# nianticlabs/implicit-depth

Measured on AMD Instinct MI355X. Metric: frames/sec (BDModel.forward hot path, 512x384, 64 planes, 8-frame tuple = 1 current + 7 source views; third-party backbones excluded), higher is better.
Workload: dtype f32

## Files before the change

implicit-depth_amd/csrc/model.hip:

```cpp
#include <cstring>
#include <vector>

#include "idh_common.h"
#include "net_plan.h"
#include "../../include/idh_model.h"

namespace {

using idh_internal::ConvStage;

constexpr int kAbi = 106;
constexpr int kHidden = 128;
constexpr int kMaxCols = 256;

inline size_t align64(size_t v) { return (v + 63) & ~(size_t)63; }

struct ColMap {
    int n;
    int col[kMaxCols];
};

__global__ __launch_bounds__(256) void pack_cols_k(const float *__restrict__ w, int ld, ColMap cols, float *__restrict__ dst, int cblocks) {
    const int total = cblocks * (kHidden / 16) * 64 * 4;
    for (int t = blockIdx.x * 256 + threadIdx.x; t < total; t += gridDim.x * 256) {
// ... 106 lines not shown
    }
    return IDH_OK;
}

uint64_t fnv(uint64_t h, const void *p, size_t n) {
    const unsigned char *c = static_cast<const unsigned char *>(p);
    for (size_t i = 0; i < n; ++i) { h ^= c[i]; h *= 1099511628211ull; }
    return h;
}

void stage_of(const idh_model_desc *d, int B, const idh_model_inputs *in, float *const *log_depth, float *const *depth, ConvStage &cs) {
    const idh_model_params *n = d->net;
    cs = ConvStage{};
    cs.enc = n->cv_blocks; cs.n_enc = 4; cs.dec = n->dec_blocks;
    cs.heads = d->kind == IDH_MODEL_DEPTH ? n->depth_heads : nullptr;
    cs.N = B; cs.H = d->H; cs.W = d->W; cs.D = d->D;
    int h = d->H, w = d->W;
    for (int i = 0; i < 4; ++i) {
        const int st = n->cv_blocks[3 * i].conv1.stride;
        if (st == 1 || st == 2) { h = (h + 2 - 3) / st + 1; w = (w + 2 - 3) / st + 1; }
        const int cimg = n->cv_blocks[3 * i + 1].conv1.cin - n->cv_blocks[3 * i].conv1.cout;
        cs.img[i + 1] = idh_tensor{in ? const_cast<float *>(in->pyramid[i + 1]) : nullptr, IDH_LAYOUT_NCHW, cimg, h, w, 0};
    }
    cs.img[0] = idh_tensor{in ? const_cast<float *>(in->pyramid[0]) : nullptr, IDH_LAYOUT_NCHW, n->dec_blocks[14].conv1.cin, 2 * cs.img[1].H, 2 * cs.img[1].W, 0};
    cs.log_depth = log_depth; cs.depth = depth;
    cs.head_mode = d->matching_input == IDH_MATCH_LAYER1_NCHW ? 1 : d->matching_input == IDH_MATCH_LAYER1_NHWC ? 2 : 0;
    cs.K = d->K;
    cs.head = n->match_head;
    cs.layer1 = in ? in->matching_layer1 : nullptr;
}
// ... 328 lines not shown
```

implicit-depth_amd/csrc/net_plan.h:

```cpp
#pragma once
#include <stddef.h>
#include <stdint.h>

#include "idh_common.h"
#include "../../include/idh_net.h"

namespace idh_internal {

enum { STAGE_SIZES = 0, STAGE_PACK = 1, STAGE_RUN = 2 };

struct ConvStage {
    const idh_block_params *enc;
    int n_enc;
    const idh_block_params *dec;
    const idh_conv_params *heads;
    int N, H, W, D;
    idh_tensor img[5];
    float *const *log_depth;
    float *const *depth;
    int head_mode;
    int K;
    const idh_conv_params *head;
    const float *layer1;
    float *cv_in;
    int cv_cs;
    const float *feat0;
    int feat0_cs, feat0_C, feat0_H, feat0_W;
    const float *match;
    int n_head_ops;
    int level_H[5], level_W[5];
// ... 12 lines not shown
```

implicit-depth_amd/csrc/networks.hip:

```cpp
#include <algorithm>
#include <array>
#include <cstring>
#include <map>
#include <tuple>
#include <vector>

#include "idh_common.h"
#include "net_plan.h"
#include "../../include/idh_net.h"
#include "../../include/idh_ops.h"

namespace {

constexpr int kWinoMinTiles = 128;
constexpr double kWinoMinFill = 0.74;
constexpr int kWino4MinTiles = 768;
constexpr double kWino4MinFill = 0.85;
constexpr long long kReuseMinBytes = 64ll << 20;
constexpr int kNarrowTileBelow = 400;
constexpr int kSplitMinChunks = 6, kSplitMax = 16;
constexpr double kProjChunkWeight = 0.5;
constexpr int kS2FirstMinBlocks = 512;
constexpr int kTargetWaves = 2048, kMinWaves = 1024;
constexpr int kTileWino = IDH_TILE_WINO, kTileWino4 = IDH_TILE_WINO4;
// ... 66 lines not shown

    float *ws_alloc(size_t floats) {
        float *p = ws_ + ws_off;
        ws_off = align64(ws_off + floats);
        if (mode_ == MODE_RUN && ws_off > ws_cap_) err = IDH_EWORKSPACE;
        return p;
    }
    float *blob_alloc(size_t floats) {
        float *p = blob_ + blob_off;
        blob_off = align64(blob_off + floats);
        return p;
    }

    View buffer(int n, int h, int w, int c) {
        const int cs_ = ceil16(c);
        if (cs_ == c) {
            auto it = free_.find(std::make_tuple(n, h, w, cs_));
            if (it != free_.end() && !it->second.empty()) {
                const int b = it->second.back();
                it->second.pop_back();
                ++recycled;
                return View{b, 0, c};
            }
        }
        Buf b{};
        b.N = n; b.H = h; b.W = w; b.cs = cs_; b.internal = true; b.zero_fill = cs_ != c;
        b.floats = (size_t)n * h * w * cs_;
        b.base = ws_alloc(b.floats);
        bufs.push_back(b);
        return View{(int)bufs.size() - 1, 0, c};
    }
    View external(const idh_tensor &t, int n) {
        Buf b{};
        b.N = n; b.H = t.H; b.W = t.W; b.cs = t.cs; b.internal = false; b.zero_fill = false;
        b.base = mode_ == MODE_RUN ? t.ptr : reinterpret_cast<float *>((uintptr_t(2) << 32) + ((uintptr_t)bufs.size() << 24));
        bufs.push_back(b);
        return View{(int)bufs.size() - 1, 0, t.C};
    }
    void release(const View &v) {
        const Buf &b = bufs[v.buf];
        if (!b.internal || v.c0 != 0 || v.C != b.cs || (long long)b.floats * 4 < kReuseMinBytes) return;
        auto &pool = free_[std::make_tuple(b.N, b.H, b.W, b.cs)];
        if (std::find(pool.begin(), pool.end(), v.buf) != pool.end()) { err = IDH_EINVAL; return; }
// ... 125 lines not shown
            if (v.C != c.cin || (c.ks != 1 && c.ks != 3) || c.cout != cout) { err = IDH_EINVAL; return out; }
            if (v.C % 16 && (v.c0 != 0 || cs(v) != ceil16(v.C))) { err = IDH_EINVAL; return out; }
            const WLayout lay = (use_wino4 && i == 0) ? W_WINO4 : (use_wino && i == 0) ? W_WINO : W_DIRECT;
            idh_conv_src &s = op.src[i];
            s.in = ptr(v); s.w = packed(c, lay); s.cs = cs(v); s.H = H(v); s.W = W(v); s.Cin = v.C;
            s.ks = c.ks; s.stride = c.stride; s.pad_mode = pad_mode;
            steps += c.ks * c.ks * (ceil16(v.C) / 16);
        }
        op.bias = bias_of(cv, cv2);
        if (res) { op.res = ptr(*res); op.res_cs = cs(*res); }
        op.out = ptr(out); op.out_cs = cs(out);
        op.Ho = Ho; op.Wo = Wo; op.Cout = cout;
        op.act = act; op.slope = slope;
        const long long M = (long long)n * Ho * Wo;
        int tm, tn, split;
        if (use_wino4) { tm = kTileWino4; tn = 0; split = 1; ++n_wino4; }
        else if (use_wino) { tm = kTileWino; tn = 0; split = 1; ++n_wino2; }
        else if (lds_eligible(srcs, cout, Wo, pad_mode)) {
            double ch = 0;
            for (const Src &s : srcs) ch += (ceil16(s.v.C) / 16) * (s.cv->ks == 3 ? 1.0 : kProjChunkWeight);
            choose_lds_tile(n, Ho, Wo, cout, (int)ch, tm, split);
            tn = lds_subtiles(cout);
            if (tn == 4 && tm == 9 && kNarrowTileBelow) {
                const long long blocks64 = (long long)n * cdiv(Ho, 4) * cdiv(Wo, 16) * (cout / 64) * split;
                if (blocks64 < kNarrowTileBelow) tn = 2;
            }
            tn = tn == 4 ? 0 : tn;
        } else if (!norm && s2_first_eligible(srcs, cout, n, Ho, Wo, pad_mode)) {
            choose_lds_tile(n, Ho, Wo, cout, ceil16(x.C) / 16, tm, split);
            tn = lds_subtiles(cout);
            tn = tn == 4 ? 0 : tn;
        } else {
            choose_tiles(M, cout, steps, tm, tn, split);
        }
        op.tile_m = tm; op.tile_n = tn; op.split_k = split;
        if (norm) {
            if ((tm != 8 && tm != 9) || tn != 1 || x2) { err = IDH_EINVAL; return out; }
            op.src[0].norm = norm->stats; op.src[0].norm_act = norm->act; op.src[0].norm_slope = norm->slope;
        }
        if (split > 1) op.ws = ws_alloc((size_t)split * M * ceil16(cout));
        ops.push_back(op);
        Meta m;
        if (res) m.reads.push_back(region(*res));
        if (norm) m.reads.push_back(Region{norm->buf, 0, 1});
        for (const Src &s : srcs) m.reads.push_back(region(s.v, true));
        m.writes.push_back(region(out));
        meta.push_back(m);
        return out;
    }
    void upsample2(const View &x, const View &out) {
        if (err) return;
        idh_op op;
        std::memset(&op, 0, sizeof op);
        op.kind = IDH_OP_UPSAMPLE2; op.N = N(x);
// ... 112 lines not shown
        const int planes = blk.conv1.cout;
        const View h = buffer(N(x), Ho, Wo, planes);
        conv(x, blk.conv1, h, IDH_ACT_LRELU, 0.2f, nullptr, nullptr, nullptr);
        const View out = out_opt ? *out_opt : buffer(N(x), Ho, Wo, planes);
        if (H(out) != Ho || W(out) != Wo) { err = IDH_EINVAL; return out; }
        if (blk.downsample.ks == 0) {
            if (x.C != planes || st != 1) { err = IDH_EINVAL; return out; }
            conv(h, blk.conv2, out, IDH_ACT_LRELU, 0.2f, &x, nullptr, nullptr);
        } else {
            conv(h, blk.conv2, out, IDH_ACT_LRELU, 0.2f, nullptr, &x, &blk.downsample);
        }
        release(h);
        return out;
    }

    static bool overlap(const std::vector<Region> &a, const std::vector<Region> &b) {
        for (const Region &x : a)
            for (const Region &y : b)
                if (x.buf == y.buf && x.c0 < y.c1 && y.c0 < x.c1) return true;
        return false;
    }
    static void launch_rank(const idh_op &op, long long r[3]) {
        r[0] = 3; r[1] = 0; r[2] = 0;
        if (op.kind == IDH_OP_CONV && op.tile_m == kTileWino) { r[0] = -1; r[1] = op.src[1].in ? 1 : 0; r[2] = -(long long)op.N * op.Ho * op.Wo * op.Cout; }
        else if (op.kind == IDH_OP_CONV && op.tile_m == 9) { r[0] = 0; r[1] = op.tile_n; }
        else if (op.kind == IDH_OP_CONV && op.tile_m == 1 && op.tile_n == 4) { r[0] = 1; }
        else if (op.kind == IDH_OP_UPSAMPLE2) { r[0] = 2; }
        else if (op.kind == IDH_OP_NCHW_TO_NHWC) { r[0] = 2; r[1] = 1; }
    }
    void schedule(int n_first = 0) {
// ... 38 lines not shown
        }
        return IDH_OK;
    }

    Mode mode() const { return mode_; }
    hipStream_t stream() const { return st_; }
    int (*before_run)(void *) = nullptr;
    void *before_ctx = nullptr;

  private:
    Mode mode_;
    float *ws_;
    size_t ws_cap_;
    float *blob_;
    hipStream_t st_;
    std::map<std::tuple<int, int, int, int>, std::vector<int>> free_;
};

bool tensor_ok(const idh_tensor *t, bool need_ptr, bool read = true) {
    if (!t || t->C <= 0 || t->H <= 0 || t->W <= 0) return false;
    if (t->layout != IDH_LAYOUT_NHWC && t->layout != IDH_LAYOUT_NCHW) return false;
    if (t->layout == IDH_LAYOUT_NHWC && (t->cs < t->C || (t->cs & 3) || (read && (t->C & 15) && t->cs != ceil16(t->C)))) return false;
    if (need_ptr && (!t->ptr || ((uintptr_t)t->ptr & 15))) return false;
    return true;
}

View input_view(Plan &p, const idh_tensor &t, int N) {
    if (t.layout == IDH_LAYOUT_NHWC) return p.external(t, N);
    const View v = p.buffer(N, t.H, t.W, t.C);
    p.import_nchw(t.ptr, N, t.C, t.H, t.W, v);
// ... 86 lines not shown
        }
        if (levels) levels->push_back(y);
        x = y;
        if (p.err) return p.err;
    }
    return p.err;
}

int build_cvencoder(Plan &p, const idh_block_params *blocks, int num_blocks, int N, const idh_tensor *cost, const idh_tensor *img, const idh_tensor *outs) {
    const bool run = p.mode() == MODE_RUN;
    if (!blocks || num_blocks <= 0 || num_blocks > 8 || N <= 0 || !tensor_ok(cost, run) || !img || !outs) return IDH_EINVAL;
    return cvencoder_body(p, blocks, num_blocks, N, input_view(p, *cost, N), img, outs, nullptr);
}

int unetpp_body(Plan &p, const idh_block_params *blocks, const idh_conv_params *heads, int N, std::vector<View> prev, const idh_tensor *fouts,
                float *const *log_depth, float *const *depth, View *feat0) {
    const bool run = p.mode() == MODE_RUN;
    const idh_block_params *out_blk[4] = {nullptr, &blocks[46], &blocks[47], &blocks[48]};
    auto want = [&](int i) { return fouts && fouts[i].C > 0; };
    std::vector<View> outputs;
    View final_v[4];
    int bi = 0;
    for (int j = 1; j <= 4; ++j) {
        for (int i = 4 - j; i >= 0; --i) {
            const idh_block_params &right = blocks[bi++], &diag = blocks[bi++];
            const bool has_up = (i + j) != 4;
            const idh_block_params *up = has_up ? &blocks[bi++] : nullptr;
            const idh_block_params &in0 = blocks[bi++], &in1 = blocks[bi++];
            const int cout = right.conv1.cout;
            const View xi = prev[i];
            const View cat = p.buffer(N, p.H(xi), p.W(xi), cout * (has_up ? 3 : 2));
            const View s0 = Plan::slice(cat, 0, cout);
            p.basic_block(xi, right, &s0);
            const View lo = p.basic_block(prev[i + 1], diag);
            if (p.H(lo) * 2 != p.H(xi) || p.W(lo) * 2 != p.W(xi)) return IDH_EINVAL;
            p.upsample2(lo, Plan::slice(cat, cout, cout));
            p.release(lo);
            if (has_up) {
                const View lo2 = p.basic_block(outputs.back(), *up);
                p.upsample2(lo2, Plan::slice(cat, 2 * cout, cout));
                p.release(lo2);
            }
            const View y0 = p.basic_block(cat, in0);
            p.release(cat);
            const bool last = j == 4 - i;
            View y;
            if (last && i == 0 && want(0) && fouts[0].layout == IDH_LAYOUT_NHWC) {
                if (!tensor_ok(&fouts[0], run) || fouts[0].C != in1.conv1.cout) return IDH_EINVAL;
                const View o = p.external(fouts[0], N);
                y = p.basic_block(y0, in1, &o);
            } else {
                y = p.basic_block(y0, in1);
                if (last && i == 0 && want(0)) {
                    if (!tensor_ok(&fouts[0], run) || fouts[0].C != in1.conv1.cout) return IDH_EINVAL;
                    p.export_nchw(y, fouts[0].ptr);
                }
            }
            p.release(y0);
            outputs.push_back(y);
            if (last) {
                if (i == 0) final_v[0] = y;
                else if (want(i)) {
                    if (!tensor_ok(&fouts[i], run) || fouts[i].C != out_blk[i]->conv1.cout) return IDH_EINVAL;
                    const View o = output_view(p, fouts[i], N);
                    final_v[i] = p.basic_block(y, *out_blk[i], &o);
                    output_done(p, fouts[i], final_v[i]);
                } else if (heads) {
                    final_v[i] = p.basic_block(y, *out_blk[i]);
                }
            }
            if (p.err) return p.err;
        }
        prev.assign(outputs.rbegin(), outputs.rend());
    }
    if (heads) {
        for (int i = 0; i < 4; ++i) {
            if (run && (!log_depth || !log_depth[i])) return IDH_EINVAL;
            p.head(final_v[i], heads[i], run ? log_depth[i] : nullptr, (run && depth) ? depth[i] : nullptr);
        }
    }
    if (feat0) *feat0 = final_v[0];
    return p.err;
}

int build_unetpp(Plan &p, const idh_block_params *blocks, int n_blocks, const idh_conv_params *heads, int N, const idh_tensor *feats,
                 const idh_tensor *fouts, float *const *log_depth, float *const *depth) {
    const bool run = p.mode() == MODE_RUN;
    if (!blocks || n_blocks != IDH_UNETPP_BLOCKS || N <= 0 || !feats) return IDH_EINVAL;
    std::vector<View> prev;
    for (int i = 0; i < 5; ++i) {
        if (!tensor_ok(&feats[i], run)) return IDH_EINVAL;
        if (i && (feats[i].H * 2 != feats[i - 1].H || feats[i].W * 2 != feats[i - 1].W)) return IDH_EINVAL;
        prev.push_back(input_view(p, feats[i], N));
    }
    return unetpp_body(p, blocks, heads, N, prev, fouts, log_depth, depth, nullptr);
}

uint64_t layout_hash(const std::vector<idh_op> &ops) {
    uint64_t h = 1469598103934665603ull;
    auto mix = [&](long long v) {
        for (int i = 0; i < 8; ++i) { h ^= (uint64_t)((v >> (8 * i)) & 0xff); h *= 1099511628211ull; }
    };
    for (const idh_op &op : ops) {
        mix(op.kind); mix(op.N); mix(op.Ho); mix(op.Wo); mix(op.Cout); mix(op.tile_m); mix(op.tile_n); mix(op.split_k); mix(op.act); mix(op.group);
        for (const idh_conv_src &s : op.src) { mix(s.Cin); mix(s.H); mix(s.W); mix(s.cs); mix(s.ks); mix(s.stride); mix(s.pad_mode); mix(s.norm != nullptr); }
    }
    return h;
}

}
// ... 42 lines not shown
        if (p.err) return p.err;
        if (p.cs(mo) != mo.C) return IDH_EUNSUPPORTED;
        s->match = p.ptr(mo);
        s->n_head_ops = (int)p.ops.size();
    }
    const View cv_in = p.buffer(s->N, s->H, s->W, s->D);
    for (int i = 0; i < 5; ++i)
        if (s->img[i].layout != IDH_LAYOUT_NCHW || !tensor_ok(&s->img[i], m == MODE_RUN)) return IDH_EINVAL;
    const View v0 = input_view(p, s->img[0], s->N);
    std::vector<View> levels{v0};
    int rc = cvencoder_body(p, s->enc, s->n_enc, s->N, cv_in, &s->img[1], nullptr, &levels);
    if (rc != IDH_OK) return rc;
    for (int i = 1; i < 5; ++i)
        if (p.H(levels[i]) * 2 != p.H(levels[i - 1]) || p.W(levels[i]) * 2 != p.W(levels[i - 1])) return IDH_EINVAL;
    View f0;
    rc = unetpp_body(p, s->dec, s->heads, s->N, levels, nullptr, s->log_depth, s->depth, &f0);
    if (rc != IDH_OK) return rc;
    s->cv_in = p.ptr(cv_in);
    s->cv_cs = p.cs(cv_in);
    s->feat0 = p.ptr(f0);
    s->feat0_cs = p.cs(f0); s->feat0_C = f0.C; s->feat0_H = p.H(f0); s->feat0_W = p.W(f0);
    for (int i = 0; i < 5; ++i) { s->level_H[i] = p.H(levels[i]); s->level_W[i] = p.W(levels[i]); }
    p.before_run = before_ops;
    p.before_ctx = ctx;
    idh_net_sizes sz{};
    if (m == MODE_PACK) return p.err;
    rc = p.finish(m == MODE_SIZES ? &sz : nullptr, s->n_head_ops);
    if (rc != IDH_OK) return rc;
    if (m == MODE_SIZES) {
        s->ws_floats = sz.workspace_floats; s->weight_floats = sz.weight_floats; s->ops = sz.ops; s->launches = sz.launches;
        s->layout_hash = layout_hash(p.ops);
// ... 54 lines not shown
                               const idh_tensor *feature_outs, float *blob, void *stream) {
    if (!blob || ((uintptr_t)blob & 255)) return IDH_EINVAL;
    Plan p(MODE_PACK, nullptr, 0, blob, idh_stream(stream));
    const int rc = build_unetpp(p, blocks, n_blocks, heads, N, feats, feature_outs, nullptr, nullptr);
    return rc != IDH_OK ? rc : p.err;
}
extern "C" int idh_unetpp_fwd(const idh_block_params *blocks, int n_blocks, const idh_conv_params *heads, const float *blob, int N,
                              const idh_tensor *feats, const idh_tensor *feature_outs, float *const *log_depth_outs, float *const *depth_outs,
                              float *ws, size_t ws_floats, void *stream) {
    if (!blob || ((uintptr_t)blob & 255) || !ws || ((uintptr_t)ws & 255)) return IDH_EINVAL;
    Plan p(MODE_RUN, ws, ws_floats, const_cast<float *>(blob), idh_stream(stream));
    const int rc = build_unetpp(p, blocks, n_blocks, heads, N, feats, feature_outs, log_depth_outs, depth_outs);
    return rc != IDH_OK ? rc : p.finish(nullptr);
}

extern "C" int idh_matching_stem_sizes(const idh_stem_params *params, int N, const idh_tensor *images, const idh_tensor *out, idh_net_sizes *sizes) {
    if (!sizes) return IDH_EINVAL;
    Plan p(MODE_SIZES, nullptr, 0, nullptr, nullptr);
    const int rc = build_matching_stem(p, params, N, images, out);
    return rc != IDH_OK ? rc : p.finish(sizes);
}
extern "C" int idh_matching_stem_pack(const idh_stem_params *params, int N, const idh_tensor *images, const idh_tensor *out, float *blob, void *stream) {
    if (!blob || ((uintptr_t)blob & 255)) return IDH_EINVAL;
    Plan p(MODE_PACK, nullptr, 0, blob, idh_stream(stream));
    const int rc = build_matching_stem(p, params, N, images, out);
    return rc != IDH_OK ? rc : p.err;
}
extern "C" int idh_matching_stem_fwd(const idh_stem_params *params, const float *blob, int N, const idh_tensor *images, const idh_tensor *out, float *ws,
                                     size_t ws_floats, void *stream) {
    if (!blob || ((uintptr_t)blob & 255) || !ws || ((uintptr_t)ws & 255)) return IDH_EINVAL;
// ... 5 lines not shown
```

implicit-depth_amd/net_abi.py:

```python
from __future__ import annotations

import ctypes as C
from typing import List, Optional, Sequence

import torch
from torch import nn

from . import _lib

LAYOUT_NHWC, LAYOUT_NCHW = 0, 1
UNETPP_BLOCKS = 49


class Tensor(C.Structure):
    _fields_ = [("ptr", C.c_void_p), ("layout", C.c_int32), ("C", C.c_int32), ("H", C.c_int32), ("W", C.c_int32), ("cs", C.c_int32)]


class ConvParams(C.Structure):
    _fields_ = [("weight", C.c_void_p), ("bias", C.c_void_p), ("cout", C.c_int32), ("cin", C.c_int32), ("ks", C.c_int32), ("stride", C.c_int32)]


class BlockParams(C.Structure):
    _fields_ = [("conv1", ConvParams), ("conv2", ConvParams), ("downsample", ConvParams)]


class NetSizes(C.Structure):
# ... 87 lines not shown


def _sigs():
    P = C.POINTER
    vp, i32, sz = C.c_void_p, C.c_int, C.c_size_t
    return {
        "idh_basic_block_sizes": (i32, [P(BlockParams), i32, P(Tensor), P(Tensor), P(NetSizes)]),
        "idh_basic_block_pack": (i32, [P(BlockParams), i32, P(Tensor), P(Tensor), vp, vp]),
        "idh_basic_block_fwd": (i32, [P(BlockParams), vp, i32, P(Tensor), P(Tensor), vp, sz, vp]),
        "idh_cvencoder_sizes": (i32, [P(BlockParams), i32, i32, P(Tensor), P(Tensor), P(Tensor), P(NetSizes)]),
        "idh_cvencoder_pack": (i32, [P(BlockParams), i32, i32, P(Tensor), P(Tensor), P(Tensor), vp, vp]),
        "idh_cvencoder_fwd": (i32, [P(BlockParams), i32, vp, i32, P(Tensor), P(Tensor), P(Tensor), vp, sz, vp]),
        "idh_unetpp_sizes": (i32, [P(BlockParams), i32, P(ConvParams), i32, P(Tensor), P(Tensor), P(NetSizes)]),
        "idh_unetpp_pack": (i32, [P(BlockParams), i32, P(ConvParams), i32, P(Tensor), P(Tensor), vp, vp]),
        "idh_unetpp_fwd": (i32, [P(BlockParams), i32, P(ConvParams), vp, i32, P(Tensor), P(Tensor), P(vp), P(vp), vp, sz, vp]),
        "idh_matching_stem_sizes": (i32, [P(StemParams), i32, P(Tensor), P(Tensor), P(NetSizes)]),
        "idh_matching_stem_pack": (i32, [P(StemParams), i32, P(Tensor), P(Tensor), vp, vp]),
        "idh_matching_stem_fwd": (i32, [P(StemParams), vp, i32, P(Tensor), P(Tensor), vp, sz, vp]),
    }


SIGS = _sigs()


def tensors(ts: Sequence[Tensor]):
    return (Tensor * len(ts))(*ts)


def ptr_array(ts: Optional[List[torch.Tensor]]):
    if ts is None:
# ... 3 lines not shown
```

implicit-depth_amd/nhwc.py:

```python
from __future__ import annotations

import ctypes as C
from dataclasses import dataclass
from typing import Dict, List, Optional, Sequence

import torch
from torch import nn

from . import _lib

OP_CONV, OP_UPSAMPLE2, OP_IMPORT, OP_EXPORT, OP_SPLITK, OP_HEAD, OP_INSTNORM, OP_UPSAMPLE2_NEAREST, OP_COPY, OP_POINTWISE_NCHW, OP_POINTWISE_UP = 1, 2, 3, 4, 5, 6, 7, 8, 9, 10, 11
OP_STEM = 12
ACT_NONE, ACT_LRELU, ACT_ELU = 0, 1, 2
PAD_ZEROS, PAD_REPLICATE = 0, 1


class ConvSrc(C.Structure):
    _fields_ = [("in_", C.c_void_p), ("w", C.c_void_p), ("cs", C.c_int32), ("H", C.c_int32), ("W", C.c_int32),
                ("Cin", C.c_int32), ("ks", C.c_int32), ("stride", C.c_int32), ("pad_mode", C.c_int32), ("_r", C.c_int32),
                ("up_in", C.c_void_p * 2), ("up_cs", C.c_int32 * 2), ("up_c0", C.c_int32), ("up_C", C.c_int32),
                ("norm", C.c_void_p), ("norm_slope", C.c_float), ("norm_act", C.c_int32)]


class Op(C.Structure):
# ... 904 lines not shown
        i_out = [p.export_nchw(o) for o in outs]
        p.schedule()
        ent = (p, i_x, i_img, i_out, outs)
        cache.put(key, ent)
    p, i_x, i_img, i_out, outs = ent
    res = [torch.empty(o.N, o.C, o.H, o.W, device=x.device, dtype=torch.float32) for o in outs]
    p.set_in(i_x, x)
    for i, f in zip(i_img, img_feats):
        p.set_in(i, f)
    for i, r in zip(i_out, res):
        p.set_out(i, r)
    p.run()
    return res


def build_decoder(p: Plan, dec, feats: List[View]):
    prev = list(feats)
    outputs: List[View] = []
    final: Dict[int, View] = {}
    for j in range(1, 5):
        for i in range(4 - j, -1, -1):
            right = dec.convs[f"right_conv_{i}{j - 1}"]
            diag = dec.convs[f"diag_conv_{i + 1}{j - 1}"]
            cout = right.conv1.out_channels
            has_up = (i + j) != 4
            xi = prev[i]
            seq = dec.convs[f"in_conv_{i}{j}"]
            fuse = (FUSE_UPSAMPLE and p.math == "fp32" and cout % 16 == 0 and xi.W >= 16 and
                    lds_eligible([(xi, seq[0].conv1)], seq[0].conv1.out_channels, xi.W, PAD_ZEROS) and seq[0].downsample is not None and
                    seq[0].downsample[0].kernel_size[0] == 1)
            if fuse:
                r = p.basic_block(xi, right)
                lo = p.basic_block(prev[i + 1], diag)
                if (lo.H * 2, lo.W * 2) != (xi.H, xi.W):
                    raise _lib.IdhError("decoder pyramid levels must differ by exactly x2")
                ups = [lo] + ([p.basic_block(outputs[-1], dec.convs[f"up_conv_{i + 1}{j}"])] if has_up else [])
                cat = CatView(r, ups)
            else:
                cat = p.buffer(xi.N, xi.H, xi.W, cout * (3 if has_up else 2))
                p.basic_block(xi, right, out=cat.slice(0, cout))
                lo = p.basic_block(prev[i + 1], diag)
                if (lo.H * 2, lo.W * 2) != (xi.H, xi.W):
                    raise _lib.IdhError("decoder pyramid levels must differ by exactly x2")
                p.upsample2(lo, cat.slice(cout, cout))
                lows = [lo]
                hold_lows = PROJ_LOWRES
                if not hold_lows:
                    p.release(lo)
                if has_up:
                    lo2 = p.basic_block(outputs[-1], dec.convs[f"up_conv_{i + 1}{j}"])
                    p.upsample2(lo2, cat.slice(2 * cout, cout))
                    lows.append(lo2)
                    if not hold_lows:
                        p.release(lo2)
            y0 = p.basic_block_upcat(cat, lows, seq[0]) if isinstance(cat, View) else None
            if y0 is None:
                y0 = p.basic_block(cat, seq[0])
            if isinstance(cat, View):
                if hold_lows:
                    for l in lows:
                        p.release(l)
                p.release(cat)
            y = p.basic_block(y0, seq.conv_0)
            p.release(y0)
            outputs.append(y)
            if j == 4 - i:
                head = dec.convs[f"output_{i}"]
                final[i] = p.basic_block(y, head[0]) if not isinstance(head[0], nn.Identity) else y
        prev = outputs[::-1]
    return final


def decoder_forward_nchw(dec, input_features: List[torch.Tensor]) -> Dict[str, torch.Tensor]:
    _check_in(*input_features)
    feats = [f.contiguous() for f in input_features]
    key = ("dec", tuple(tuple(f.shape) for f in feats), str(feats[0].device), _param_key(dec))
    cache = _plan_cache(dec)
    ent = cache.get(key)
    if ent is None:
        p = Plan(feats[0].device, math=math_of(dec))
        views, i_in = [], []
        for f in feats:
            v = p.buffer(f.shape[0], f.shape[2], f.shape[3], f.shape[1])
# ... 226 lines not shown
    final: Dict[int, View] = {}
    for bi, blk in enumerate((dec.block1, dec.block2, dec.block3, dec.block4)):
        skip = feats[-2 - bi]
        cout = blk.pre_concat_conv.conv2.out_channels
        y = _conv_block(p, x, blk.pre_concat_conv)
        if (y.H * 2, y.W * 2) != (skip.H, skip.W):
            raise _lib.IdhError("decoder pyramid levels must differ by exactly x2")
        cat = p.buffer(skip.N, skip.H, skip.W, cout + skip.C)
        p.upsample2(y, cat.slice(0, cout), nearest=True)
        p.copy(skip, cat.slice(cout, skip.C))
        x = _conv_block(p, cat, blk.post_concat_conv)
        final[3 - bi] = x
    return final


def build_any_decoder(p: Plan, dec, feats: List[View]) -> Dict[int, View]:
    if hasattr(dec, "block1"):
        return build_skip_decoder(p, dec, feats)
    return build_decoder(p, dec, feats)


def build_regression_heads(p: Plan, dec, final: Dict[int, View]) -> Dict[int, "tuple"]:
    heads = {}
    for i, seq in ((3, dec.out1), (2, dec.out2), (1, dec.out3), (0, dec.out4)):
        v = final[i]
        h1 = p.buffer(v.N, v.H, v.W, seq[0].out_channels)
        p.conv(v, seq[0], h1, act=ACT_ELU)
        h2 = p.buffer(v.N, v.H, v.W, seq[2].out_channels)
        p.conv(h1, seq[2], h2, act=ACT_ELU)
        heads[i] = (h2, seq[4])
    return heads


def skip_regression_forward_nchw(dec, input_features: List[torch.Tensor]) -> Dict[str, torch.Tensor]:
# ... 34 lines not shown
```

implicit-depth_amd/pipeline.py:

```python
from __future__ import annotations

from typing import Dict, List, Optional, Sequence

import torch
from torch import nn

from . import _lib, nhwc
from .cost_volume import CostVolumeManager, ZeroCostVolumeManager, volume_opts
from .mlp import occlusion_logits


class HotPath(nn.Module):

    def __init__(self, cost_volume: nn.Module, cost_volume_net: nn.Module, depth_decoder: nn.Module,
                 binary_mlp: Optional[nn.Module] = None, min_depth: float = 0.25, max_depth: float = 5.0,
                 conv_math: Optional[str] = None, matching_model: Optional[nn.Module] = None):
        super().__init__()
        self.conv_math = conv_math
        self.cost_volume = cost_volume
        self.cost_volume_net = cost_volume_net
        self.depth_decoder = depth_decoder
        self.binary_mlp = binary_mlp
        self.matching_model = matching_model
        self.min_depth, self.max_depth = float(min_depth), float(max_depth)
        self.thresholder = None
        self._plans = nhwc.PlanCache()
        _lib.watch_state_dict_loads(self)

    def _plan(self, B, K, C, H, W, enc_shapes: Sequence[Sequence[int]], device, head: Optional[str] = None, head_ch: int = 0,
              images: Optional[torch.Tensor] = None):
        geom = None
        if head == "images":
            _, shape, strides = nhwc.image_strides(images)
            geom = (tuple(shape), strides)
        key = (B, K, C, H, W, tuple(tuple(s) for s in enc_shapes), str(device), self.conv_math, head, head_ch, geom,
               nhwc._param_key(self.cost_volume_net), nhwc._param_key(self.depth_decoder),
               nhwc.ParamKey(nhwc._param_key(self.matching_model.net[5]) + nhwc._param_key(self.matching_model.net[8])) if head else None,
               nhwc.stem_param_key(self.matching_model.net[:5]) if head == "images" else None)
        ent = self._plans.get(key)
        if ent is not None:
            return ent
        D = self.cost_volume.num_depth_bins
        p = nhwc.Plan(device, math=self.conv_math)
        st = {"lowest": None, "planes": torch.empty(D, device=device)}
        ent = {"plan": p, "state": st, "heads": {}, "i_l1": None}
        if head is None:
            st["cur_n"] = torch.empty(B, H, W, C, device=device)
            st["src_n"] = torch.empty(B, K, H, W, C, device=device)
            ent["feats"] = (st["cur_n"].data_ptr(), st["src_n"].data_ptr(), (B, K, C, H, W), 0, 0)
        else:
# ... 11 lines not shown
            else:
                x = nhwc.View(torch.empty(1, device=device).expand(M, H, W, head_ch), 0, head_ch)
                y = nhwc.build_matching_head(p, self.matching_model, x)
                ent["i_l1"] = n0
            if y.C != C:
                raise _lib.IdhError(f"matching head produces {y.C} channels, cost volume expects {C}")
            hw = H * W * C
            ent["feats"] = (y.ptr, y.ptr + 4 * hw, (B, K, C, H, W), (K + 1) * hw, (K + 1) * hw)
            ent["match_view"] = y
        n_pre = len(p.ops)
        cv_in = p.buffer(B, H, W, D)
        v0 = p.buffer(B, enc_shapes[0][2], enc_shapes[0][3], enc_shapes[0][1])
        i_enc = [p.import_nchw(enc_shapes[0], v0)]
        outs, i_img = nhwc.build_cv_encoder(p, self.cost_volume_net, cv_in, enc_shapes[1:])
        i_enc += i_img
        final = nhwc.build_any_decoder(p, self.depth_decoder, [v0] + outs)
        ent.update(cv_in=cv_in, i_enc=i_enc, final=final)
        if getattr(self.depth_decoder, "depth_head", False):
            for i, v in final.items():
                ent["heads"][i] = p.head(v, self.depth_decoder.convs[f"output_{i}"][1], torch.empty(1, device=device))
        elif hasattr(self.depth_decoder, "out1"):
            for i, (hv, last) in nhwc.build_regression_heads(p, self.depth_decoder, final).items():
                ent["heads"][i] = p.head(hv, last, torch.empty(1, device=device))
        ent["n_head_ops"] = p.schedule_segments(n_pre)
        return self._plans.put(key, ent)

    def forward(self, matching_cur_feats: Optional[torch.Tensor], matching_src_feats: Optional[torch.Tensor], cur_feats: List[torch.Tensor],
                src_cam_T_cur_cam: torch.Tensor, cur_cam_T_src_cam: torch.Tensor, src_K: torch.Tensor, cur_invK: torch.Tensor,
                rendered_depth: Optional[torch.Tensor] = None, prior: Optional[torch.Tensor] = None,
                return_mask: bool = False, return_features: bool = False,
                prior_inputs: Optional[Dict[str, torch.Tensor]] = None, infer_depth: bool = False,
# ... 24 lines not shown
            if matching_layer1.dim() != 5:
                raise _lib.IdhError(f"matching_layer1 must be (B, K+1, C, H, W), got {tuple(matching_layer1.shape)}")
            B, K1, head_ch, H, W = matching_layer1.shape
            K, C = K1 - 1, self.matching_model.net[8].out_channels
            l1 = matching_layer1.reshape(B * K1, head_ch, H, W)
            if l1.is_contiguous():
                head = "nchw"
            elif l1.is_contiguous(memory_format=torch.channels_last):
                head = "nhwc"
            else:
                l1, head = l1.contiguous(), "nchw"
        else:
            B, K, C, H, W = matching_src_feats.shape
        dev = src_K.device
        cur_feats = [f if f.is_contiguous() else f.contiguous() for f in cur_feats]
        ent = self._plan(B, K, C, H, W, [f.shape for f in cur_feats], dev, head, head_ch, images)
        p, st = ent["plan"], ent["state"]
        L = _lib.lib()
        sp = _lib.stream_ptr()
        D = self.cost_volume.num_depth_bins
        out: Dict[str, torch.Tensor] = {}

        zero_volume = isinstance(self.cost_volume, ZeroCostVolumeManager)
        if head is not None:
            p.set_in(ent["i_l1"], l1)
            p.run(0, ent["n_head_ops"])
        elif not zero_volume:
            mc = matching_cur_feats if matching_cur_feats.is_contiguous() else matching_cur_feats.contiguous()
            ms = matching_src_feats if matching_src_feats.is_contiguous() else matching_src_feats.contiguous()
            _lib.check(L.idh_nchw_to_nhwc_f32(mc.data_ptr(), st["cur_n"].data_ptr(), B, C, H * W, sp), "idh_nchw_to_nhwc_f32")
            _lib.check(L.idh_nchw_to_nhwc_f32(ms.data_ptr(), st["src_n"].data_ptr(), B * K, C, H * W, sp), "idh_nchw_to_nhwc_f32")
# ... 94 lines not shown
```

include/idh_net.h:

```cpp
#ifndef IDH_NET_H_
#define IDH_NET_H_

#include <stddef.h>
#include <stdint.h>

#ifdef __cplusplus
extern "C" {
#endif
#if defined(__GNUC__) || defined(__clang__)
#pragma GCC visibility push(default)
#endif

#define IDH_LAYOUT_NHWC 0
#define IDH_LAYOUT_NCHW 1

typedef struct idh_tensor {
    float *ptr;
    int32_t layout;
    int32_t C, H, W;
    int32_t cs;
} idh_tensor;

typedef struct idh_conv_params {
    const float *weight;
// ... 23 lines not shown
                        const idh_tensor *outs, idh_net_sizes *sizes);
int idh_cvencoder_pack(const idh_block_params *blocks, int num_blocks, int N, const idh_tensor *cost, const idh_tensor *img_feats,
                       const idh_tensor *outs, float *weight_blob, void *stream);
int idh_cvencoder_fwd(const idh_block_params *blocks, int num_blocks, const float *weight_blob, int N, const idh_tensor *cost,
                      const idh_tensor *img_feats, const idh_tensor *outs, float *workspace, size_t workspace_floats, void *stream);

#define IDH_UNETPP_BLOCKS 49
int idh_unetpp_sizes(const idh_block_params *blocks, int n_blocks, const idh_conv_params *heads, int N, const idh_tensor *feats,
                     const idh_tensor *feature_outs, idh_net_sizes *sizes);
int idh_unetpp_pack(const idh_block_params *blocks, int n_blocks, const idh_conv_params *heads, int N, const idh_tensor *feats,
                    const idh_tensor *feature_outs, float *weight_blob, void *stream);
int idh_unetpp_fwd(const idh_block_params *blocks, int n_blocks, const idh_conv_params *heads, const float *weight_blob, int N,
                   const idh_tensor *feats, const idh_tensor *feature_outs, float *const *log_depth_outs, float *const *depth_outs,
                   float *workspace, size_t workspace_floats, void *stream);

typedef struct idh_bn_params {
    const float *weight, *bias, *running_mean, *running_var;
    float eps;
    int32_t _r;
} idh_bn_params;

typedef struct idh_stem_params {
    const float *conv1_weight;
    idh_bn_params bn1;
    const float *layer1_conv[4];
    idh_bn_params layer1_bn[4];
} idh_stem_params;

int idh_matching_stem_sizes(const idh_stem_params *params, int N, const idh_tensor *images, const idh_tensor *out, idh_net_sizes *sizes);
int idh_matching_stem_pack(const idh_stem_params *params, int N, const idh_tensor *images, const idh_tensor *out, float *weight_blob, void *stream);
// ... 11 lines not shown
```

Before: 680.9.

## Skip unused coarse-scale decoder output blocks and release low-res inputs early

Adds a scale mask to the UNet++ decoder so the output_i blocks for coarse scales are skipped when only the finest scale is consumed (non-depth model, or Python pipeline when no features are returned). A dry-run reservation path keeps weight-blob packing offsets stable while no kernels are emitted. It also releases intermediate pyramid inputs earlier, so workspace buffers can be recycled. The risk is that it drops outputs some callers may need when the mask is misapplied.

```diff
diff --git a/implicit-depth_amd/csrc/model.hip b/implicit-depth_amd/csrc/model.hip
--- a/implicit-depth_amd/csrc/model.hip
+++ b/implicit-depth_amd/csrc/model.hip
@@ -144,6 +144,7 @@
     cs = ConvStage{};
     cs.enc = n->cv_blocks; cs.n_enc = 4; cs.dec = n->dec_blocks;
     cs.heads = d->kind == IDH_MODEL_DEPTH ? n->depth_heads : nullptr;
+    cs.scales = d->kind == IDH_MODEL_DEPTH ? IDH_SCALES_ALL : 0x1;
     cs.N = B; cs.H = d->H; cs.W = d->W; cs.D = d->D;
     int h = d->H, w = d->W;
     for (int i = 0; i < 4; ++i) {
diff --git a/implicit-depth_amd/csrc/net_plan.h b/implicit-depth_amd/csrc/net_plan.h
--- a/implicit-depth_amd/csrc/net_plan.h
+++ b/implicit-depth_amd/csrc/net_plan.h
@@ -14,6 +14,7 @@
     int n_enc;
     const idh_block_params *dec;
     const idh_conv_params *heads;
+    unsigned scales;
     int N, H, W, D;
     idh_tensor img[5];
     float *const *log_depth;
diff --git a/implicit-depth_amd/csrc/networks.hip b/implicit-depth_amd/csrc/networks.hip
--- a/implicit-depth_amd/csrc/networks.hip
+++ b/implicit-depth_amd/csrc/networks.hip
@@ -104,6 +104,7 @@
 
     View buffer(int n, int h, int w, int c) {
         const int cs_ = ceil16(c);
+        if (dry_) return phantom(n, h, w, c, cs_);
         if (cs_ == c) {
             auto it = free_.find(std::make_tuple(n, h, w, cs_));
             if (it != free_.end() && !it->second.empty()) {
@@ -117,6 +118,13 @@
         b.N = n; b.H = h; b.W = w; b.cs = cs_; b.internal = true; b.zero_fill = cs_ != c;
         b.floats = (size_t)n * h * w * cs_;
         b.base = ws_alloc(b.floats);
+        bufs.push_back(b);
+        return View{(int)bufs.size() - 1, 0, c};
+    }
+    View phantom(int n, int h, int w, int c, int cs_) {
+        Buf b{};
+        b.N = n; b.H = h; b.W = w; b.cs = cs_; b.internal = false; b.zero_fill = false;
+        b.base = reinterpret_cast<float *>((uintptr_t(7) << 32) + ((uintptr_t)bufs.size() << 24));
         bufs.push_back(b);
         return View{(int)bufs.size() - 1, 0, c};
     }
@@ -272,8 +280,8 @@
         op.act = act; op.slope = slope;
         const long long M = (long long)n * Ho * Wo;
         int tm, tn, split;
-        if (use_wino4) { tm = kTileWino4; tn = 0; split = 1; ++n_wino4; }
-        else if (use_wino) { tm = kTileWino; tn = 0; split = 1; ++n_wino2; }
+        if (use_wino4) { tm = kTileWino4; tn = 0; split = 1; n_wino4 += !dry_; }
+        else if (use_wino) { tm = kTileWino; tn = 0; split = 1; n_wino2 += !dry_; }
         else if (lds_eligible(srcs, cout, Wo, pad_mode)) {
             double ch = 0;
             for (const Src &s : srcs) ch += (ceil16(s.v.C) / 16) * (s.cv->ks == 3 ? 1.0 : kProjChunkWeight);
@@ -296,6 +304,7 @@
             if ((tm != 8 && tm != 9) || tn != 1 || x2) { err = IDH_EINVAL; return out; }
             op.src[0].norm = norm->stats; op.src[0].norm_act = norm->act; op.src[0].norm_slope = norm->slope;
         }
+        if (dry_) return out;
         if (split > 1) op.ws = ws_alloc((size_t)split * M * ceil16(cout));
         ops.push_back(op);
         Meta m;
@@ -438,6 +447,18 @@
         return out;
     }
 
+    void reserve_block(const View &x, const idh_block_params &blk, int out_cs) {
+        dry_ = true;
+        if (out_cs) {
+            const int st = blk.conv1.stride == 2 ? 2 : 1;
+            const View o = phantom(N(x), (H(x) + 2 - 3) / st + 1, (W(x) + 2 - 3) / st + 1, blk.conv1.cout, out_cs);
+            basic_block(x, blk, &o);
+        } else {
+            basic_block(x, blk);
+        }
+        dry_ = false;
+    }
+
     static bool overlap(const std::vector<Region> &a, const std::vector<Region> &b) {
         for (const Region &x : a)
             for (const Region &y : b)
@@ -506,6 +527,7 @@
     size_t ws_cap_;
     float *blob_;
     hipStream_t st_;
+    bool dry_ = false;
     std::map<std::tuple<int, int, int, int>, std::vector<int>> free_;
 };
 
@@ -622,10 +644,13 @@
 }
 
 int unetpp_body(Plan &p, const idh_block_params *blocks, const idh_conv_params *heads, int N, std::vector<View> prev, const idh_tensor *fouts,
-                float *const *log_depth, float *const *depth, View *feat0) {
+                float *const *log_depth, float *const *depth, View *feat0, unsigned scales = IDH_SCALES_ALL, bool keep_slots = false) {
     const bool run = p.mode() == MODE_RUN;
+    if ((scales & ~(unsigned)IDH_SCALES_ALL) || (heads && scales != IDH_SCALES_ALL)) return IDH_EINVAL;
     const idh_block_params *out_blk[4] = {nullptr, &blocks[46], &blocks[47], &blocks[48]};
-    auto want = [&](int i) { return fouts && fouts[i].C > 0; };
+    auto sel = [&](int i) { return ((scales >> i) & 1u) != 0; };
+    auto given = [&](int i) { return fouts && fouts[i].C > 0; };
+    auto want = [&](int i) { return given(i) && sel(i); };
     std::vector<View> outputs;
     View final_v[4];
     int bi = 0;
@@ -642,6 +667,7 @@
             p.basic_block(xi, right, &s0);
             const View lo = p.basic_block(prev[i + 1], diag);
             if (p.H(lo) * 2 != p.H(xi) || p.W(lo) * 2 != p.W(xi)) return IDH_EINVAL;
+            if (j > 1 && !has_up) p.release(prev[i + 1]);
             p.upsample2(lo, Plan::slice(cat, cout, cout));
             p.release(lo);
             if (has_up) {
@@ -668,7 +694,9 @@
             outputs.push_back(y);
             if (last) {
                 if (i == 0) final_v[0] = y;
-                else if (want(i)) {
+                else if (!sel(i)) {
+                    if (keep_slots && given(i)) p.reserve_block(y, *out_blk[i], fouts[i].layout == IDH_LAYOUT_NHWC ? fouts[i].cs : 0);
+                } else if (want(i)) {
                     if (!tensor_ok(&fouts[i], run) || fouts[i].C != out_blk[i]->conv1.cout) return IDH_EINVAL;
                     const View o = output_view(p, fouts[i], N);
                     final_v[i] = p.basic_block(y, *out_blk[i], &o);
@@ -692,7 +720,7 @@
 }
 
 int build_unetpp(Plan &p, const idh_block_params *blocks, int n_blocks, const idh_conv_params *heads, int N, const idh_tensor *feats,
-                 const idh_tensor *fouts, float *const *log_depth, float *const *depth) {
+                 const idh_tensor *fouts, float *const *log_depth, float *const *depth, unsigned scales = IDH_SCALES_ALL) {
     const bool run = p.mode() == MODE_RUN;
     if (!blocks || n_blocks != IDH_UNETPP_BLOCKS || N <= 0 || !feats) return IDH_EINVAL;
     std::vector<View> prev;
@@ -701,7 +729,7 @@
         if (i && (feats[i].H * 2 != feats[i - 1].H || feats[i].W * 2 != feats[i - 1].W)) return IDH_EINVAL;
         prev.push_back(input_view(p, feats[i], N));
     }
-    return unetpp_body(p, blocks, heads, N, prev, fouts, log_depth, depth, nullptr);
+    return unetpp_body(p, blocks, heads, N, prev, fouts, log_depth, depth, nullptr, scales, true);
 }
 
 uint64_t layout_hash(const std::vector<idh_op> &ops) {
@@ -774,7 +802,7 @@
     for (int i = 1; i < 5; ++i)
         if (p.H(levels[i]) * 2 != p.H(levels[i - 1]) || p.W(levels[i]) * 2 != p.W(levels[i - 1])) return IDH_EINVAL;
     View f0;
-    rc = unetpp_body(p, s->dec, s->heads, s->N, levels, nullptr, s->log_depth, s->depth, &f0);
+    rc = unetpp_body(p, s->dec, s->heads, s->N, levels, nullptr, s->log_depth, s->depth, &f0, s->scales);
     if (rc != IDH_OK) return rc;
     s->cv_in = p.ptr(cv_in);
     s->cv_cs = p.cs(cv_in);
@@ -859,6 +887,31 @@
     return rc != IDH_OK ? rc : p.finish(nullptr);
 }
 
+extern "C" int idh_unetpp_sizes_ex(const idh_block_params *blocks, int n_blocks, const idh_conv_params *heads, int N, const idh_tensor *feats,
+                                   const idh_tensor *feature_outs, uint32_t scales, idh_net_sizes *sizes) {
+    if (!sizes) return IDH_EINVAL;
+    Plan p(MODE_SIZES, nullptr, 0, nullptr, nullptr);
+    const int rc = build_unetpp(p, blocks, n_blocks, heads, N, feats, feature_outs, nullptr, nullptr, scales);
+    return rc != IDH_OK ? rc : p.finish(sizes);
+}
+extern "C" int idh_unetpp_pack_ex(const idh_block_params *blocks, int n_blocks, const idh_conv_params *heads, int N, const idh_tensor *feats,
+                                  const idh_tensor *feature_outs, uint32_t scales, float *blob, void *stream) {
+    if (!blob || ((uintptr_t)blob & 255)) return IDH_EINVAL;
+    Plan p(MODE_PACK, nullptr, 0, blob, idh_stream(stream));
+    const int rc = build_unetpp(p, blocks, n_blocks, heads, N, feats, feature_outs, nullptr, nullptr, scales);
+    return rc != IDH_OK ? rc : p.err;
+}
+extern "C" int idh_unetpp_fwd_ex(const idh_block_params *blocks, int n_blocks, const idh_conv_params *heads, const float *blob, size_t weight_floats,
+                                 int N, const idh_tensor *feats, const idh_tensor *feature_outs, uint32_t scales, float *const *log_depth_outs,
+                                 float *const *depth_outs, float *ws, size_t ws_floats, void *stream) {
+    if (!blob || ((uintptr_t)blob & 255) || !ws || ((uintptr_t)ws & 255)) return IDH_EINVAL;
+    Plan p(MODE_RUN, ws, ws_floats, const_cast<float *>(blob), idh_stream(stream));
+    const int rc = build_unetpp(p, blocks, n_blocks, heads, N, feats, feature_outs, log_depth_outs, depth_outs, scales);
+    if (rc != IDH_OK) return rc;
+    if (weight_floats != p.blob_off) return IDH_EINVAL;
+    return p.finish(nullptr);
+}
+
 extern "C" int idh_matching_stem_sizes(const idh_stem_params *params, int N, const idh_tensor *images, const idh_tensor *out, idh_net_sizes *sizes) {
     if (!sizes) return IDH_EINVAL;
     Plan p(MODE_SIZES, nullptr, 0, nullptr, nullptr);
diff --git a/implicit-depth_amd/net_abi.py b/implicit-depth_amd/net_abi.py
--- a/implicit-depth_amd/net_abi.py
+++ b/implicit-depth_amd/net_abi.py
@@ -10,6 +10,7 @@
 
 LAYOUT_NHWC, LAYOUT_NCHW = 0, 1
 UNETPP_BLOCKS = 49
+SCALES_ALL = 0xF
 
 
 class Tensor(C.Structure):
@@ -127,6 +128,9 @@
         "idh_unetpp_sizes": (i32, [P(BlockParams), i32, P(ConvParams), i32, P(Tensor), P(Tensor), P(NetSizes)]),
         "idh_unetpp_pack": (i32, [P(BlockParams), i32, P(ConvParams), i32, P(Tensor), P(Tensor), vp, vp]),
         "idh_unetpp_fwd": (i32, [P(BlockParams), i32, P(ConvParams), vp, i32, P(Tensor), P(Tensor), P(vp), P(vp), vp, sz, vp]),
+        "idh_unetpp_sizes_ex": (i32, [P(BlockParams), i32, P(ConvParams), i32, P(Tensor), P(Tensor), C.c_uint32, P(NetSizes)]),
+        "idh_unetpp_pack_ex": (i32, [P(BlockParams), i32, P(ConvParams), i32, P(Tensor), P(Tensor), C.c_uint32, vp, vp]),
+        "idh_unetpp_fwd_ex": (i32, [P(BlockParams), i32, P(ConvParams), vp, sz, i32, P(Tensor), P(Tensor), C.c_uint32, P(vp), P(vp), vp, sz, vp]),
         "idh_matching_stem_sizes": (i32, [P(StemParams), i32, P(Tensor), P(Tensor), P(NetSizes)]),
         "idh_matching_stem_pack": (i32, [P(StemParams), i32, P(Tensor), P(Tensor), vp, vp]),
         "idh_matching_stem_fwd": (i32, [P(StemParams), vp, i32, P(Tensor), P(Tensor), vp, sz, vp]),
diff --git a/implicit-depth_amd/nhwc.py b/implicit-depth_amd/nhwc.py
--- a/implicit-depth_amd/nhwc.py
+++ b/implicit-depth_amd/nhwc.py
@@ -942,7 +942,10 @@
     return res
 
 
-def build_decoder(p: Plan, dec, feats: List[View]):
+ALL_SCALES = 0b1111
+
+
+def build_decoder(p: Plan, dec, feats: List[View], scales: int = ALL_SCALES):
     prev = list(feats)
     outputs: List[View] = []
     final: Dict[int, View] = {}
@@ -970,6 +973,8 @@
                 lo = p.basic_block(prev[i + 1], diag)
                 if (lo.H * 2, lo.W * 2) != (xi.H, xi.W):
                     raise _lib.IdhError("decoder pyramid levels must differ by exactly x2")
+                if j > 1 and not has_up:
+                    p.release(prev[i + 1])
                 p.upsample2(lo, cat.slice(cout, cout))
                 lows = [lo]
                 hold_lows = PROJ_LOWRES
@@ -994,7 +999,10 @@
             outputs.append(y)
             if j == 4 - i:
                 head = dec.convs[f"output_{i}"]
-                final[i] = p.basic_block(y, head[0]) if not isinstance(head[0], nn.Identity) else y
+                if isinstance(head[0], nn.Identity):
+                    final[i] = y
+                elif (scales >> i) & 1:
+                    final[i] = p.basic_block(y, head[0])
         prev = outputs[::-1]
     return final
 
@@ -1251,10 +1259,10 @@
     return final
 
 
-def build_any_decoder(p: Plan, dec, feats: List[View]) -> Dict[int, View]:
+def build_any_decoder(p: Plan, dec, feats: List[View], scales: int = ALL_SCALES) -> Dict[int, View]:
     if hasattr(dec, "block1"):
         return build_skip_decoder(p, dec, feats)
-    return build_decoder(p, dec, feats)
+    return build_decoder(p, dec, feats, scales)
 
 
 def build_regression_heads(p: Plan, dec, final: Dict[int, View]) -> Dict[int, "tuple"]:
diff --git a/implicit-depth_amd/pipeline.py b/implicit-depth_amd/pipeline.py
--- a/implicit-depth_amd/pipeline.py
+++ b/implicit-depth_amd/pipeline.py
@@ -27,13 +27,19 @@
         self._plans = nhwc.PlanCache()
         _lib.watch_state_dict_loads(self)
 
+    def _scales(self, return_features: bool) -> int:
+        dec = self.depth_decoder
+        if return_features or self.binary_mlp is None or getattr(dec, "depth_head", False) or hasattr(dec, "out1"):
+            return nhwc.ALL_SCALES
+        return 0b0001
+
     def _plan(self, B, K, C, H, W, enc_shapes: Sequence[Sequence[int]], device, head: Optional[str] = None, head_ch: int = 0,
-              images: Optional[torch.Tensor] = None):
+              images: Optional[torch.Tensor] = None, scales: int = nhwc.ALL_SCALES):
         geom = None
         if head == "images":
             _, shape, strides = nhwc.image_strides(images)
             geom = (tuple(shape), strides)
-        key = (B, K, C, H, W, tuple(tuple(s) for s in enc_shapes), str(device), self.conv_math, head, head_ch, geom,
+        key = (B, K, C, H, W, tuple(tuple(s) for s in enc_shapes), str(device), self.conv_math, head, head_ch, geom, scales,
                nhwc._param_key(self.cost_volume_net), nhwc._param_key(self.depth_decoder),
                nhwc.ParamKey(nhwc._param_key(self.matching_model.net[5]) + nhwc._param_key(self.matching_model.net[8])) if head else None,
                nhwc.stem_param_key(self.matching_model.net[:5]) if head == "images" else None)
@@ -75,7 +81,7 @@
         i_enc = [p.import_nchw(enc_shapes[0], v0)]
         outs, i_img = nhwc.build_cv_encoder(p, self.cost_volume_net, cv_in, enc_shapes[1:])
         i_enc += i_img
-        final = nhwc.build_any_decoder(p, self.depth_decoder, [v0] + outs)
+        final = nhwc.build_any_decoder(p, self.depth_decoder, [v0] + outs, scales)
         ent.update(cv_in=cv_in, i_enc=i_enc, final=final)
         if getattr(self.depth_decoder, "depth_head", False):
             for i, v in final.items():
@@ -130,7 +136,7 @@
             B, K, C, H, W = matching_src_feats.shape
         dev = src_K.device
         cur_feats = [f if f.is_contiguous() else f.contiguous() for f in cur_feats]
-        ent = self._plan(B, K, C, H, W, [f.shape for f in cur_feats], dev, head, head_ch, images)
+        ent = self._plan(B, K, C, H, W, [f.shape for f in cur_feats], dev, head, head_ch, images, self._scales(return_features))
         p, st = ent["plan"], ent["state"]
         L = _lib.lib()
         sp = _lib.stream_ptr()
diff --git a/include/idh_net.h b/include/idh_net.h
--- a/include/idh_net.h
+++ b/include/idh_net.h
@@ -61,6 +61,15 @@
                    const idh_tensor *feats, const idh_tensor *feature_outs, float *const *log_depth_outs, float *const *depth_outs,
                    float *workspace, size_t workspace_floats, void *stream);
 
+#define IDH_SCALES_ALL 0xF
+int idh_unetpp_sizes_ex(const idh_block_params *blocks, int n_blocks, const idh_conv_params *heads, int N, const idh_tensor *feats,
+                        const idh_tensor *feature_outs, uint32_t scales, idh_net_sizes *sizes);
+int idh_unetpp_pack_ex(const idh_block_params *blocks, int n_blocks, const idh_conv_params *heads, int N, const idh_tensor *feats,
+                       const idh_tensor *feature_outs, uint32_t scales, float *weight_blob, void *stream);
+int idh_unetpp_fwd_ex(const idh_block_params *blocks, int n_blocks, const idh_conv_params *heads, const float *weight_blob, size_t weight_floats,
+                      int N, const idh_tensor *feats, const idh_tensor *feature_outs, uint32_t scales, float *const *log_depth_outs,
+                      float *const *depth_outs, float *workspace, size_t workspace_floats, void *stream);
+
 typedef struct idh_bn_params {
     const float *weight, *bias, *running_mean, *running_var;
     float eps;
```

Result: faster. 688.8, median of 6 (+1.2%).
